# zarrs/zarrs

Hardware: AMD Instinct MI355X
Metric: decoded-array GiB/s, device-resident chunks, 1/2/4/8 MI355X; % HBM roofline (higher is better)
Workload: dtype f32; 1 GPU; C2: 4096 independent 64^3 f32 chunks per GPU, [transpose{order:[2,1,0]}, bytes{endian:big}], device-resident; chunks_per_gpu=4096, parallelism=chunk-partitioned x1

## Files before the change

include/zgpu.h:

```cpp
#ifndef ZGPU_H
#define ZGPU_H

#include <stdint.h>

#ifdef __cplusplus
extern "C" {
#endif

#define ZGPU_MAX_DIMS 8

enum {
  ZGPU_OK = 0,
  ZGPU_INVALID_CHECKSUM = 1,
  ZGPU_DECODED_SIZE_MISMATCH = 2,
  ZGPU_SHARD_INDEX_OOB = 3,
  ZGPU_CORRUPT_STREAM = 4,
  ZGPU_INVALID_BYTE_RANGE = 5,
  ZGPU_UNSUPPORTED = 6,
  ZGPU_CRC_INPUT_TOO_SHORT = 7,
  ZGPU_SHARD_TOO_SMALL = 8,
  ZGPU_SHUFFLE_LENGTH = 9,
  ZGPU_INVALID_ARGUMENT = 10,
  ZGPU_HIP_ERROR = 11,
  ZGPU_STORAGE_ERROR = 12,
// ... 46 lines not shown
  uint64_t shape[ZGPU_MAX_DIMS];
} zgpu_out_view;

#define ZGPU_COALESCE 0x20u

int zgpu_decode_into(zgpu_chain *chain, uint32_t ndim, const zgpu_chunk_desc *descs, uint64_t n,
                     const zgpu_out_view *view, uint32_t flags, int32_t *status, void *hip_stream);

typedef struct zgpu_result zgpu_result;
int zgpu_decode_pinned(zgpu_chain *chain, uint32_t ndim, const zgpu_chunk_desc *descs, uint64_t n,
                       const uint64_t *out_shape, uint32_t flags, int32_t *status, const void **data,
                       zgpu_result **result);
void zgpu_result_release(zgpu_result *result);

int zgpu_ctx_set_coalescing(zgpu_ctx *ctx, uint32_t window_us, uint32_t max_calls, uint64_t max_bytes);
int zgpu_ctx_coalescing_stats(const zgpu_ctx *ctx, uint64_t *batches, uint64_t *calls);

int zgpu_plan_create(zgpu_chain *chain, uint32_t ndim, const zgpu_chunk_desc *descs, uint64_t n,
                     const uint64_t *out_shape, uint32_t flags, zgpu_plan **out);
int zgpu_plan_execute(zgpu_plan *plan, void *out, int32_t *status, void *hip_stream);
int zgpu_plan_status(zgpu_plan *plan, int32_t *status, void *hip_stream);
void zgpu_plan_destroy(zgpu_plan *plan);
uint64_t zgpu_plan_algorithmic_bytes(const zgpu_plan *plan);

typedef struct zgpu_group zgpu_group;
int zgpu_group_create(zgpu_chain *const *chains, uint32_t ndim, uint32_t n_parts, const zgpu_chunk_desc *const *descs,
                      const uint64_t *n_descs, const uint64_t *const *out_shapes, uint32_t flags, zgpu_group **out);
int zgpu_group_execute(zgpu_group *group, void *const *outs, int32_t *status, void *hip_stream);
int zgpu_group_status(zgpu_group *group, int32_t *status, void *hip_stream);
uint32_t zgpu_group_layout(const zgpu_group *group, uint32_t *lane_of, uint32_t *part_of, uint32_t *lits_first,
                           uint32_t n);
uint64_t zgpu_group_algorithmic_bytes(const zgpu_group *group);
uint32_t zgpu_group_counters(const zgpu_group *group, uint64_t *out, uint32_t n);
void zgpu_group_destroy(zgpu_group *group);

#define ZGPU_CTR_ENC_BYTES 0
#define ZGPU_CTR_ZSTD_SERIAL 1
#define ZGPU_CTR_ZSTD_PARALLEL 2
#define ZGPU_CTR_BLOSC_RERUN 3
#define ZGPU_CTR_BLOSC_BLOCKS 4
#define ZGPU_CTR_ITEMS 5
#define ZGPU_CTR_ZSTD_LATENCY 6
#define ZGPU_N_COUNTERS 7
uint32_t zgpu_plan_counters(const zgpu_plan *plan, uint64_t *out, uint32_t n);
uint32_t zgpu_last_counters(uint64_t *out, uint32_t n);

// ... 82 lines not shown
```

zarrs_amd/_lib.py:

```python
from __future__ import annotations

import ctypes as C
import os

HERE = os.path.dirname(os.path.abspath(__file__))
LIB_PATH = os.environ.get("ZGPU_LIB") or os.path.join(HERE, "lib", "libzgpu.so")
MAX_DIMS = 8

STATUS_NAMES = [
    "OK", "INVALID_CHECKSUM", "DECODED_SIZE_MISMATCH", "SHARD_INDEX_OOB", "CORRUPT_STREAM",
    "INVALID_BYTE_RANGE", "UNSUPPORTED", "CRC_INPUT_TOO_SHORT", "SHARD_TOO_SMALL", "SHUFFLE_LENGTH",
    "INVALID_ARGUMENT", "HIP_ERROR", "STORAGE_ERROR",
]
OK, INVALID_CHECKSUM, DECODED_SIZE_MISMATCH, SHARD_INDEX_OOB, CORRUPT_STREAM, INVALID_BYTE_RANGE, \
    UNSUPPORTED, CRC_INPUT_TOO_SHORT, SHARD_TOO_SMALL, SHUFFLE_LENGTH, INVALID_ARGUMENT, HIP_ERROR, \
    STORAGE_ERROR = range(13)

ENC_DEVICE = 0x1
OUT_DEVICE = 0x2
ONE_STREAM = 0x10
ZSTD_LITS_FIRST = 0x40
NO_VALIDATE = 0x4
DIRECT_IO = 0x8
COALESCE = 0x20
WHOLE = (1 << 64) - 1

EXPORTS = [
    "zgpu_ctx_create", "zgpu_ctx_destroy", "zgpu_last_error", "zgpu_status_name", "zgpu_version",
    "zgpu_chain_create", "zgpu_chain_destroy", "zgpu_chain_element_size", "zgpu_decode_batch",
    "zgpu_plan_create", "zgpu_plan_execute", "zgpu_plan_status", "zgpu_plan_destroy", "zgpu_plan_algorithmic_bytes",
    "zgpu_retrieve_array_subset", "zgpu_decode_files", "zgpu_retrieve_array_subset_files",
    "zgpu_chain_encoded_size", "zgpu_encode_batch", "zgpu_plan_counters", "zgpu_last_counters",
    "zgpu_last_size_mismatch", "zgpu_cache_create", "zgpu_cache_destroy", "zgpu_cache_clear", "zgpu_cache_stats",
    "zgpu_cache_retrieve_array_subset", "zgpu_retrieve_array_subset_dlpack", "zgpu_chain_encoded_bound",
    "zgpu_encode_chunks", "zgpu_retrieve_array_subset_multi", "zgpu_decode_into", "zgpu_ctx_set_coalescing",
    "zgpu_ctx_coalescing_stats", "zgpu_ctx_refcount", "zgpu_decode_pinned", "zgpu_result_release",
    "zgpu_encode_pinned", "zgpu_ctx_release_cached", "zgpu_ctx_pool_stats",
    "zgpu_group_create", "zgpu_group_execute", "zgpu_group_status", "zgpu_group_layout",
    "zgpu_group_algorithmic_bytes", "zgpu_group_counters", "zgpu_group_destroy",
]
CTR_ENC_BYTES, CTR_ZSTD_SERIAL, CTR_ZSTD_PARALLEL, CTR_BLOSC_RERUN, CTR_BLOSC_BLOCKS, CTR_ITEMS, \
    CTR_ZSTD_LATENCY = range(7)
N_COUNTERS = 7


class ChunkDesc(C.Structure):
    _fields_ = [
        ("enc", C.c_void_p),
        ("enc_len", C.c_uint64),
        ("chunk_shape", C.c_uint64 * MAX_DIMS),
        ("sel_start", C.c_uint64 * MAX_DIMS),
        ("sel_shape", C.c_uint64 * MAX_DIMS),
        ("out_start", C.c_uint64 * MAX_DIMS),
    ]


class OutView(C.Structure):
    _fields_ = [
        ("base", C.c_void_p),
        ("array_shape", C.c_uint64 * MAX_DIMS),
        ("start", C.c_uint64 * MAX_DIMS),
        ("shape", C.c_uint64 * MAX_DIMS),
    ]
# ... 63 lines not shown
    L.zgpu_ctx_refcount.argtypes = [vp]
    L.zgpu_ctx_refcount.restype = C.c_int64
    L.zgpu_last_error.restype = C.c_char_p
    L.zgpu_last_error.argtypes = [vp]
    L.zgpu_status_name.restype = C.c_char_p
    L.zgpu_status_name.argtypes = [i32]
    L.zgpu_version.restype = C.c_char_p
    L.zgpu_chain_create.argtypes = [vp, C.c_char_p, C.c_char_p, vp, u32, i32, C.POINTER(vp)]
    L.zgpu_chain_destroy.argtypes = [vp]
    L.zgpu_chain_element_size.restype = u32
    L.zgpu_chain_element_size.argtypes = [vp]
    L.zgpu_decode_batch.argtypes = [vp, u32, C.POINTER(ChunkDesc), u64, vp, P64, u32,
                                    C.POINTER(C.c_int32), vp]
    L.zgpu_decode_into.argtypes = [vp, u32, C.POINTER(ChunkDesc), u64, C.POINTER(OutView), u32,
                                   C.POINTER(C.c_int32), vp]
    L.zgpu_ctx_set_coalescing.argtypes = [vp, u32, u32, u64]
    L.zgpu_ctx_coalescing_stats.argtypes = [vp, P64, P64]
    L.zgpu_plan_create.argtypes = [vp, u32, C.POINTER(ChunkDesc), u64, P64, u32, C.POINTER(vp)]
    L.zgpu_plan_execute.argtypes = [vp, vp, C.POINTER(C.c_int32), vp]
    L.zgpu_plan_status.argtypes = [vp, C.POINTER(C.c_int32), vp]
    L.zgpu_plan_destroy.argtypes = [vp]
    L.zgpu_plan_algorithmic_bytes.restype = u64
    L.zgpu_plan_algorithmic_bytes.argtypes = [vp]
    L.zgpu_group_create.argtypes = [C.POINTER(vp), u32, u32, C.POINTER(C.POINTER(ChunkDesc)), P64, C.POINTER(P64),
                                    u32, C.POINTER(vp)]
    L.zgpu_group_execute.argtypes = [vp, C.POINTER(vp), C.POINTER(C.c_int32), vp]
    L.zgpu_group_status.argtypes = [vp, C.POINTER(C.c_int32), vp]
    L.zgpu_group_layout.restype = u32
    L.zgpu_group_layout.argtypes = [vp, C.POINTER(u32), C.POINTER(u32), C.POINTER(u32), u32]
    L.zgpu_group_algorithmic_bytes.restype = u64
    L.zgpu_group_algorithmic_bytes.argtypes = [vp]
    L.zgpu_group_counters.restype = u32
    L.zgpu_group_counters.argtypes = [vp, P64, u32]
    L.zgpu_group_destroy.argtypes = [vp]
    L.zgpu_retrieve_array_subset.argtypes = [vp, u32, P64, P64, C.POINTER(vp), P64, P64, P64, vp,
                                             u32, vp]
    L.zgpu_decode_files.argtypes = [vp, u32, C.POINTER(ChunkDesc), C.POINTER(FileRange), u64, vp, P64,
                                    u32, C.POINTER(C.c_int32), vp]
    L.zgpu_retrieve_array_subset_files.argtypes = [vp, u32, P64, P64, C.POINTER(C.c_char_p), P64, P64,
                                                   vp, u32, vp]
    L.zgpu_chain_encoded_size.restype = C.c_int64
    L.zgpu_chain_encoded_size.argtypes = [vp, u32, P64]
    L.zgpu_encode_batch.argtypes = [vp, u32, P64, vp, P64, C.POINTER(EncodeDesc), u64, u32, vp]
    L.zgpu_chain_encoded_bound.restype = C.c_int64
    L.zgpu_chain_encoded_bound.argtypes = [vp, u32, P64]
    L.zgpu_encode_chunks.argtypes = [vp, u32, P64, vp, P64, C.POINTER(EncodeDesc), u64, u32, P64, vp]
# ... 45 lines not shown
```

zarrs_amd/csrc/kernels/dev.hpp:

```cpp
#pragma once
#include <hip/hip_runtime.h>

#include <cstdint>

namespace zgpu {

__device__ __forceinline__ uint32_t swap_word(uint32_t x, uint32_t comp) {
  if (comp == 4) return __builtin_bswap32(x);
  if (comp == 2) return ((x >> 8) & 0x00FF00FFu) | ((x << 8) & 0xFF00FF00u);
  return x;
}

__device__ __forceinline__ uint4 swap_vec(uint4 v, uint32_t comp) {
  if (comp == 8) return make_uint4(__builtin_bswap32(v.y), __builtin_bswap32(v.x),
                                   __builtin_bswap32(v.w), __builtin_bswap32(v.z));
  return make_uint4(swap_word(v.x, comp), swap_word(v.y, comp), swap_word(v.z, comp),
                    swap_word(v.w, comp));
}

typedef unsigned int zg_v4u __attribute__((ext_vector_type(4)));
__device__ __forceinline__ uint4 nt_load16(const void *p) {
  const zg_v4u x = __builtin_nontemporal_load((const zg_v4u *)p);
  return make_uint4(x.x, x.y, x.z, x.w);
}
__device__ __forceinline__ void nt_store16(void *p, uint4 v) {
  const zg_v4u x = {v.x, v.y, v.z, v.w};
  __builtin_nontemporal_store(x, (zg_v4u *)p);
}

}
```

zarrs_amd/csrc/kernels/launch.hpp:

```cpp
#pragma once
#include <hip/hip_runtime.h>

#include "../common.hpp"

#include <cstdlib>

namespace zgpu {

inline uint64_t max_grid_blocks(uint32_t threads) {
  uint64_t m = (0xFFFFFFFFull / threads) & ~(uint64_t)0xFFF;
  if (const char *e = std::getenv("ZGPU_MAX_GRID")) {
    const uint64_t v = std::strtoull(e, nullptr, 10);
    if (v && v < m) m = v;
  }
  return m;
}

inline uint32_t device_cu_count() {
  static uint32_t cache[64] = {0};
  int dev = 0;
  if (hipGetDevice(&dev) != hipSuccess || dev < 0 || dev >= 64) return 256;
  if (!cache[dev]) {
    int n = 0;
    if (hipDeviceGetAttribute(&n, hipDeviceAttributeMultiprocessorCount, dev) != hipSuccess || n <= 0) n = 256;
    cache[dev] = (uint32_t)n;
  }
  return cache[dev];
}

enum ScatterMode : uint32_t { SCATTER_ROWS = 0, SCATTER_TILED = 1, SCATTER_GENERIC = 2 };
constexpr __host__ __device__ int tiled_slabs(uint32_t es) { return es == 8 ? 2 : 4; }

hipError_t launch_scatter(const ZgItem *items, const uint64_t *geom, uint32_t *status, const ZgScatter &P,
                          uint8_t *out, uint32_t n_items, uint32_t mode, uint64_t units_per_item,
                          hipStream_t s, uint32_t *live_scratch = nullptr);
uint64_t scatter_units_per_item(uint32_t mode, const ZgScatter &P, const uint64_t *max_sel_shape);

struct ZgBoxCopy {
  uint32_t outer, pad0;
  uint64_t shape[ZG_MAXD], src_stride[ZG_MAXD], dst_stride[ZG_MAXD];
  uint64_t src_base, dst_base, run_bytes, n_runs;
};
hipError_t launch_box_copy(const uint8_t *src, uint8_t *dst, const ZgBoxCopy &P, hipStream_t s);

hipError_t launch_crc32c_strip(ZgItem *items, uint32_t *status, uint32_t n_items, int at_start, int verify,
                               hipStream_t s);

enum : uint32_t { CK_ADLER32 = 0, CK_FLETCHER32 = 1 };
uint64_t linsum_scratch_bytes(uint32_t n_items, uint64_t len_hint);
hipError_t launch_linsum_strip(uint32_t kind, ZgItem *items, uint32_t *status, uint32_t n_items, int at_start,
                               int verify, uint64_t len_hint, void *scratch, hipStream_t s);

struct ZgIndexSpec {
  uint64_t n_inner;
  uint64_t index_bytes;
  uint32_t at_start;
  uint32_t big_endian;
  uint32_t n_crc;
  uint32_t crc_at_start[4];
// ... 188 lines not shown
```

zarrs_amd/csrc/kernels/scatter.hip:

```cpp
#include <hip/hip_runtime.h>

#include <algorithm>

#include "../common.hpp"
#include "launch.hpp"
#include "dev.hpp"

namespace zgpu {

__device__ __forceinline__ uint4 load_elem(const uint8_t *p, uint32_t es, uint32_t comp, uint32_t swap) {
  uint8_t b[16];
  uintptr_t a = (uintptr_t)p;
  if (es == 4 && (a & 3) == 0) {
    uint32_t w = *(const uint32_t *)p;
    if (swap) w = swap_word(w, comp);
    return make_uint4(w, 0, 0, 0);
  }
  if (es == 2 && (a & 1) == 0) {
    uint32_t w = *(const uint16_t *)p;
    if (swap) w = ((w >> 8) | (w << 8)) & 0xFFFFu;
    return make_uint4(w, 0, 0, 0);
  }
  if (es == 8 && (a & 7) == 0) {
    uint2 w = *(const uint2 *)p;
// ... 241 lines not shown
  rows_unit(items, geom, status, P, out, (uint32_t)(bid / blocks_per_item), (uint32_t)(bid % blocks_per_item));
}

__global__ void k_live_items(const ZgItem *__restrict__ items, const uint32_t *__restrict__ status, uint32_t n,
                             uint32_t *__restrict__ list, uint32_t *__restrict__ count) {
  const uint32_t i = blockIdx.x * blockDim.x + threadIdx.x;
  if (i < n && !status[i] && !(items[i].flags & ZG_ITEM_DIRECT)) list[atomicAdd(count, 1u)] = i;
}

__global__ __launch_bounds__(SCATTER_THREADS) void k_scatter_rows_list(
    const ZgItem *__restrict__ items, const uint64_t *__restrict__ geom, uint32_t *__restrict__ status,
    ZgScatter P, uint8_t *__restrict__ out, uint32_t blocks_per_item, const uint32_t *__restrict__ list,
    const uint32_t *__restrict__ count) {
  const uint64_t total = (uint64_t)*count * blocks_per_item;
  for (uint64_t w = blockIdx.x; w < total; w += gridDim.x) {
    __syncthreads();
    rows_unit(items, geom, status, P, out, list[w / blocks_per_item], (uint32_t)(w % blocks_per_item));
  }
}

constexpr int TILE = 64;

template <int ES>
__global__ __launch_bounds__(SCATTER_THREADS) void k_scatter_tiled(
    const ZgItem *__restrict__ items, const uint64_t *__restrict__ geom, uint32_t *__restrict__ status,
    ZgScatter P, uint8_t *__restrict__ out, uint32_t tiles_per_item, uint64_t block_base) {
  using T = typename std::conditional<ES == 1, uint8_t, typename std::conditional<ES == 2, uint16_t,
            typename std::conditional<ES == 4, uint32_t, uint2>::type>::type>::type;
  constexpr int TJ = tiled_slabs(ES);
  constexpr int PITCH = TILE + (ES >= 4 ? 1 : 4 / ES);
  constexpr int SLAB = TILE * PITCH + (ES >= 4 ? 1 : 4 / ES);
  __shared__ T tile[TJ * SLAB];
  const uint64_t bid = block_base + blockIdx.x;
  const uint32_t item = (uint32_t)(bid / tiles_per_item);
  uint32_t t = (uint32_t)(bid % tiles_per_item);
  const ZgItem it = items[item];
  if (!item_live(it, status, item, P)) return;
  const uint32_t nd = P.nd, A = P.tile_a, Lx = nd - 1, B = P.tile_b;
  const uint64_t *g = geom + (uint64_t)item * 3 * nd;
  const uint64_t *ss = g, *sh = g + nd, *os = g + 2 * nd;
  const bool hasB = B < nd;
  const uint64_t bext = hasB ? sh[B] : 1;
  const uint32_t nta = (uint32_t)((sh[A] + TILE - 1) / TILE), ntl = (uint32_t)((sh[Lx] + TILE - 1) / TILE);
  const uint32_t nbg = (uint32_t)((bext + TJ - 1) / TJ);
  const uint32_t ta = t % nta; t /= nta;
  const uint32_t tl = t % ntl; t /= ntl;
  const uint32_t tb = t % nbg; t /= nbg;
  uint64_t so = 0, dof = 0, rem = t;
  for (int d = (int)nd - 1; d >= 0; d--) {
    if ((uint32_t)d == A || (uint32_t)d == Lx || (uint32_t)d == B) continue;
    const uint64_t c = rem % sh[d];
    rem /= sh[d];
    so += (ss[d] + c) * P.enc_stride[d];
    dof += (os[d] + c) * P.out_stride[d];
  }
  if (rem) return;
  const uint64_t a0 = (uint64_t)ta * TILE, l0 = (uint64_t)tl * TILE, b0 = (uint64_t)tb * TJ;
  const uint32_t na = (uint32_t)min<uint64_t>(TILE, sh[A] - a0), nl = (uint32_t)min<uint64_t>(TILE, sh[Lx] - l0);
  const uint32_t nb = (uint32_t)min<uint64_t>(TJ, bext - b0);
  const uint64_t sL = P.enc_stride[Lx], dA = P.out_stride[A];
  const uint64_t sB = hasB ? P.enc_stride[B] : 0, dB = hasB ? P.out_stride[B] : 0;
  so += (ss[A] + a0) * P.enc_stride[A] + (ss[Lx] + l0) * sL + (hasB ? (ss[B] + b0) * sB : 0);
  dof += (os[A] + a0) * dA + (os[Lx] + l0) + (hasB ? (os[B] + b0) * dB : 0);
  T *dst = (T *)(out) + dof;
  constexpr int VPR = TILE * ES / 16;
  constexpr int EPV = 16 / ES;
  constexpr int NV = TJ * TILE * VPR;
  const bool oaligned = (((uint64_t)dst & 15) == 0) && ((dA * ES) % 16 == 0) && ((dB * ES) % 16 == 0) &&
                        nl == TILE;
  if (it.flags & ZG_ITEM_FILL) {
    T fv;
    __builtin_memcpy(&fv, P.fill, ES);
    if (oaligned) {
      uint4 x;
      T *xe = (T *)&x;
#pragma unroll
      for (int k = 0; k < EPV; k++) xe[k] = fv;
      for (uint32_t e = threadIdx.x; e < (uint32_t)NV; e += SCATTER_THREADS) {
        const uint32_t a = e / (TJ * VPR), jj = (e / VPR) % TJ, v = e % VPR;
        if (a < na && jj < nb) nt_store16(dst + jj * dB + (uint64_t)a * dA + v * EPV, x);
      }
    } else {
      for (uint32_t e = threadIdx.x; e < (uint32_t)(TJ * TILE * TILE); e += SCATTER_THREADS) {
        const uint32_t a = e / (TJ * TILE), jj = (e / TILE) % TJ, l = e % TILE;
        if (a < na && jj < nb && l < nl) dst[jj * dB + (uint64_t)a * dA + l] = fv;
      }
    }
    return;
  }
  const T *src = (const T *)(it.src) + so;
  const uint32_t swap = P.swap && P.comp > 1;
  const bool aligned = (((uint64_t)src & 15) == 0) && ((sL * ES) % 16 == 0) && ((sB * ES) % 16 == 0) &&
                       na == TILE;
  if (aligned) {
    constexpr int PER = NV / SCATTER_THREADS;
    uint4 x[PER];
#pragma unroll
    for (int p = 0; p < PER; p++) {
      const uint32_t e = p * SCATTER_THREADS + threadIdx.x;
      const uint32_t l = e / (TJ * VPR), jj = (e / VPR) % TJ, v = e % VPR;
      if (l < nl && jj < nb) x[p] = nt_load16(src + jj * sB + (uint64_t)l * sL + v * EPV);
    }
#pragma unroll
    for (int p = 0; p < PER; p++) {
      const uint32_t e = p * SCATTER_THREADS + threadIdx.x;
      const uint32_t l = e / (TJ * VPR), jj = (e / VPR) % TJ, v = e % VPR;
      if (l < nl && jj < nb) {
        uint4 y = swap ? swap_vec(x[p], P.comp) : x[p];
        const T *ye = (const T *)&y;
#pragma unroll
        for (int k = 0; k < EPV; k++) tile[jj * SLAB + l * PITCH + v * EPV + k] = ye[k];
      }
    }
  } else {
    for (uint32_t e = threadIdx.x; e < (uint32_t)(TJ * TILE * TILE); e += SCATTER_THREADS) {
      const uint32_t l = e / (TJ * TILE), jj = (e / TILE) % TJ, a = e % TILE;
      if (l < nl && jj < nb && a < na) {
        uint4 y = load_elem((const uint8_t *)(src + jj * sB + (uint64_t)l * sL + a), ES, P.comp, swap);
        T v;
        __builtin_memcpy(&v, &y, ES);
        tile[jj * SLAB + l * PITCH + a] = v;
      }
    }
  }
  __syncthreads();
  if (oaligned) {
#pragma unroll
    for (int p = 0; p < NV / SCATTER_THREADS; p++) {
      const uint32_t e = p * SCATTER_THREADS + threadIdx.x;
      const uint32_t a = e / (TJ * VPR), jj = (e / VPR) % TJ, v = e % VPR;
      if (a < na && jj < nb) {
        uint4 y;
        T *ye = (T *)&y;
#pragma unroll
        for (int k = 0; k < EPV; k++) ye[k] = tile[jj * SLAB + (v * EPV + k) * PITCH + a];
        nt_store16(dst + jj * dB + (uint64_t)a * dA + v * EPV, y);
      }
    }
  } else {
    for (uint32_t e = threadIdx.x; e < (uint32_t)(TJ * TILE * TILE); e += SCATTER_THREADS) {
      const uint32_t a = e / (TJ * TILE), jj = (e / TILE) % TJ, l = e % TILE;
      if (a < na && jj < nb && l < nl) dst[jj * dB + (uint64_t)a * dA + l] = tile[jj * SLAB + l * PITCH + a];
    }
  }
}

__global__ __launch_bounds__(SCATTER_THREADS) void k_scatter_generic(
    const ZgItem *__restrict__ items, const uint64_t *__restrict__ geom, uint32_t *__restrict__ status,
    ZgScatter P, uint8_t *__restrict__ out, uint32_t blocks_per_item, uint64_t block_base) {
  const uint64_t bid = block_base + blockIdx.x;
  const uint32_t item = (uint32_t)(bid / blocks_per_item);
  const uint32_t blk = (uint32_t)(bid % blocks_per_item);
  const ZgItem it = items[item];
  if (!item_live(it, status, item, P)) return;
  const uint32_t nd = P.nd, es = P.es;
  const uint64_t *g = geom + (uint64_t)item * 3 * nd;
  uint64_t n = 1;
  for (uint32_t d = 0; d < nd; d++) n *= g[nd + d];
  const uint64_t e = (uint64_t)blk * SCATTER_THREADS + threadIdx.x;
  if (e >= n) return;
  uint64_t rem = e, so = 0, dof = 0;
  for (int d = (int)nd - 1; d >= 0; d--) {
    const uint64_t c = rem % g[nd + d];
    rem /= g[nd + d];
    so += (g[d] + c) * P.enc_stride[d];
// ... 69 lines not shown

uint64_t scatter_units_per_item(uint32_t mode, const ZgScatter &P, const uint64_t *max_sel_shape) {
  const uint32_t nd = P.nd;
  if (mode == SCATTER_ROWS) {
    uint64_t rows = 1;
    for (uint32_t d = 0; d + 1 < nd; d++) rows *= max_sel_shape[d];
    return (rows + ROWS_PER_BLOCK - 1) / ROWS_PER_BLOCK;
  }
  if (mode == SCATTER_TILED) {
    const uint64_t tj = tiled_slabs(P.es);
    uint64_t t = 1;
    for (uint32_t d = 0; d < nd; d++) {
      if (d == P.tile_a || d == nd - 1) t *= (max_sel_shape[d] + TILE - 1) / TILE;
      else if (d == P.tile_b) t *= (max_sel_shape[d] + tj - 1) / tj;
      else t *= max_sel_shape[d];
    }
    return t;
  }
  uint64_t n = 1;
  for (uint32_t d = 0; d < nd; d++) n *= max_sel_shape[d];
  return (n + SCATTER_THREADS - 1) / SCATTER_THREADS;
}

}

namespace zgpu {

__global__ __launch_bounds__(64) void k_box_copy(const uint8_t *__restrict__ src, uint8_t *__restrict__ dst,
                                                   ZgBoxCopy P) {
  const uint32_t lane = threadIdx.x & 63;
  const uint64_t waves = (uint64_t)gridDim.x * (blockDim.x >> 6);
  for (uint64_t r = (uint64_t)blockIdx.x * (blockDim.x >> 6) + (threadIdx.x >> 6); r < P.n_runs; r += waves) {
    uint64_t k = r, so = 0, dof = 0;
    for (int d = (int)P.outer - 1; d >= 0; d--) {
      const uint64_t c = k % P.shape[d];
      k /= P.shape[d];
      so += c * P.src_stride[d];
      dof += c * P.dst_stride[d];
    }
    const uint8_t *s = src + P.src_base + so;
    uint8_t *t = dst + P.dst_base + dof;
    const uint64_t n = P.run_bytes;
    if ((((uintptr_t)s | (uintptr_t)t | n) & 15) == 0) {
      for (uint64_t i = (uint64_t)lane * 16; i < n; i += 64 * 16)
        *(uint4 *)(t + i) = *(const uint4 *)(s + i);
    } else if ((((uintptr_t)s | (uintptr_t)t | n) & 3) == 0) {
// ... 17 lines not shown
```

zarrs_amd/csrc/zgpu.cpp:

```cpp
#include <hip/hip_runtime.h>

#include <algorithm>
#include <atomic>
#include <chrono>
#include <cstdio>
#include <cstdlib>
#include <cstring>
#include <condition_variable>
#include <map>
#include <memory>
#include <mutex>
#include <string>
#include <vector>

#include "../../include/zgpu.h"
#include "chain.hpp"
#include "common.hpp"
#include "kernels/launch.hpp"
#include "fsstore.hpp"
#include "internal.hpp"
#include "xfer.hpp"

using namespace zgpu;

// ... 307 lines not shown
    Z.ev_done = zev2[1];
  }
  struct Grow {
    void *p = nullptr;
    size_t n = 0;
  };
  Grow bl_info, bl_bases, bl_subs, bl_sub_status, bl_sub_kind, bl_blocks, bl_tmp, bl_zblks, bl_znblk, bl_zmode,
      bl_zlit, bl_zseq, bl_zaux, bl_zser, bl_lzl, bl_zseg, bl_zrec, bl_zalias, bl_znorm, gz_crc, live_list,
      ck_parts;
  uint64_t in_len_hint = 0;
  uint8_t *bl_h = nullptr;
  size_t bl_h_n = 0;
  void *grow(Grow &g, size_t bytes) {
    if (g.n < bytes) {
      ctx->dev_free(g.p);
      g.p = ctx->dev_alloc(bytes);
      g.n = bytes;
    }
    return g.p;
  }
  unsigned long long *d_counter = nullptr;
  uint8_t *d_ctl = nullptr, *h_ctl = nullptr;
  size_t ctl_bytes = 0;
  uint8_t *d_enc_stage = nullptr;
  uint64_t last_enc_bytes = 0;
  uint64_t last_counters[CTR_N] = {};
  uint8_t *last_out = nullptr;
  BlCaps bl_caps{};
  bool bl_caps_valid = false, bl_caps_seen = false;
  bool bl_direct = false;
  bool gz_direct = false;
  GzDirect gz{};
  std::vector<uint64_t> bl_need;
  uint64_t *d_bl_need = nullptr;
  bool zstd_serial_off = false, zstd_serial_skipped = false;
  uint32_t *d_zser = nullptr;
  uint32_t *d_order = nullptr;
  uint32_t *d_gz_seg = nullptr;
  bool no_scatter = false;

  ~zgpu_plan() {
    if (!ctx) return;
    struct Unref {
      zgpu_ctx *c;
      ~Unref() { ctx_unref(c); }
    } unref{ctx};
    if (own.stream) {
      (void)hipStreamSynchronize(own.stream);
      (void)hipStreamDestroy(own.stream);
    }
    if (own.order_ev) (void)hipEventDestroy(own.order_ev);
    void *bufs[] = {d_items, d_items_init, d_geom, d_shards, d_index, d_shard_status, d_mids, d_mids_init,
                    d_mid_status, d_shard_status2, d_mid_shards, d_index2, d_bl_need,
                    d_pool[0], d_pool[1], zs.blks, zs.nblk, zs.mode, zs.lit, zs.seq, d_ctl,
                    d_enc_stage, d_zser, d_order, d_gz_seg, zs.lit_rec, zs.ext, zs.ext_cnt, zs.norm};
    for (void *b : bufs) ctx->dev_free(b);
    if (zside) {
      (void)hipStreamSynchronize(zside);
      (void)hipStreamDestroy(zside);
    }
    if (zs2) {
      (void)hipStreamSynchronize(zs2);
      (void)hipStreamDestroy(zs2);
    }
    for (hipEvent_t e : zev2)
      if (e) (void)hipEventDestroy(e);
    for (hipEvent_t e : zev)
      if (e) (void)hipEventDestroy(e);
    for (Grow *g : {&bl_info, &bl_bases, &bl_subs, &bl_sub_status, &bl_sub_kind, &bl_blocks, &bl_tmp, &bl_zblks,
                    &bl_znblk, &bl_zmode, &bl_zlit, &bl_zseq, &bl_zaux, &bl_zser, &bl_lzl, &bl_zseg, &bl_zrec, &bl_zalias,
                    &bl_znorm, &gz_crc, &live_list, &ck_parts})
      ctx->dev_free(g->p);
    ctx->host_free(bl_h);
    ctx->host_free(h_ctl);
  }
};

static void reset_call_state() {
// ... 335 lines not shown
    s *= eshape[a];
  }
  for (uint32_t a = 0; a < nd; a++) S.enc_stride[m[a]] = est[a];
  for (uint32_t d = 0; d < nd; d++) {
    S.chunk_shape[d] = leaf_shape[d];
    S.out_stride[d] = out_strides[mo[d]];
  }
  S.tile_a = m[nd - 1];
  S.tile_b = ZG_MAXD;
  for (uint32_t d = 0; d + 1 < nd; d++) {
    if (d == S.tile_a) continue;
    if (S.tile_b == ZG_MAXD || S.enc_stride[d] <= S.enc_stride[S.tile_b]) S.tile_b = d;
  }
  if (outer_perm && S.out_stride[nd - 1] != 1) {
    P.scatter_mode = SCATTER_GENERIC;
  } else if (S.tile_a == nd - 1) {
    P.scatter_mode = SCATTER_ROWS;
  } else if (!S.shuffle && (S.es == 1 || S.es == 2 || S.es == 4 || S.es == 8)) {
    P.scatter_mode = SCATTER_TILED;
  } else {
    P.scatter_mode = SCATTER_GENERIC;
  }
  P.scatter_units = P.items.empty() ? 0 : scatter_units_per_item(P.scatter_mode, S, max_sel);

  if (!P.stages.empty() && P.stages.back().kind == ST_BLOSC && P.scatter_mode == SCATTER_ROWS && !S.swap &&
      !S.shuffle && S.nelem > 0 && S.out_stride[nd - 1] == 1 && (S.chunk_shape[nd - 1] * S.es) % 16 == 0) {
    bool ok = true;
    uint64_t st = 1;
    for (int a = (int)nd - 1; a >= 0 && ok; a--) {
      ok = S.enc_stride[a] == st && (a == (int)nd - 1 || (S.out_stride[a] * S.es) % 16 == 0);
      st *= S.chunk_shape[a];
    }
    for (size_t i = 0; i < P.items.size() && ok; i++) {
      if (P.items[i].flags & ZG_ITEM_FILL) continue;
      const uint64_t *g = P.geom.data() + i * 3 * nd;
      for (uint32_t d = 0; d < nd && ok; d++) ok = g[d] == 0 && g[nd + d] == S.chunk_shape[d];
      ok = ok && (g[2 * nd + nd - 1] * S.es) % 16 == 0;
    }
    P.bl_direct = ok && !std::getenv("ZGPU_BLOSC_NO_DIRECT");
  }
  {
    const char *gz_env = std::getenv("ZGPU_GZIP_DIRECT");
    const bool gz_on = !gz_env || std::atoi(gz_env) != 0;
    const uint64_t Lb = S.chunk_shape[nd - 1] * S.es;
    bool ok = gz_on && !P.stages.empty() && P.stages.back().kind == ST_GZIP && P.scatter_mode == SCATTER_ROWS &&
              !S.swap && !S.shuffle && S.nelem > 0 && nd >= 1 && nd <= 3 && S.out_stride[nd - 1] == 1 && Lb >= 16 &&
// ... 77 lines not shown
        if (ni * P.slot_bytes <= par_max) {
          P.zs.ext = (uint32_t *)C.dev_alloc(2 * ni * P.slot_bytes * 4);
          P.zs.ext_cnt = (unsigned long long *)C.dev_alloc(ZEXT_ROUNDS * 8);
          P.zs.ext_items = ni;
        }
      }
    }
  }
  P.in_len_hint = 0;
  if (P.sharded) {
    uint64_t shard_max = 0;
    for (const ZgShard &sh : P.shards) shard_max = std::max(shard_max, sh.len);
    const int64_t b = P.leaf ? chain_encoded_bound(*P.leaf, P.scatter.nelem) : -1;
    P.in_len_hint = b >= 0 ? std::min<uint64_t>((uint64_t)b, shard_max) : shard_max;
  } else {
    for (const ZgItem &it : P.items) P.in_len_hint = std::max(P.in_len_hint, it.len);
  }
  for (const Stage &s : P.stages)
    if (ni && (s.kind == ST_ADLER32 || s.kind == ST_FLETCHER32))
      P.grow(P.ck_parts, linsum_scratch_bytes((uint32_t)ni, std::max(P.in_len_hint, P.slot_bytes)));
  P.ctl_bytes = 256 + ni * 4;
  P.d_ctl = (uint8_t *)C.dev_alloc(P.ctl_bytes);
  P.h_ctl = (uint8_t *)C.host_alloc(P.ctl_bytes);
  P.d_counter = (unsigned long long *)P.d_ctl;
  P.d_status = (uint32_t *)(P.d_ctl + 256);
  P.zs.counters = P.d_counter + CTR_ZSTD_SERIAL;
  P.zs.lat_count = P.d_counter + CTR_ZSTD_LATENCY;
  P.zs.ser_count = P.d_counter + CTR_ZSTD_NSER;
  P.zs.max_nblk = P.d_counter + CTR_ZSTD_MAXBLK;
  if (const char *e = std::getenv("ZGPU_ZSTD_FORCE_SERIAL")) P.zs.force_serial = std::atoi(e) != 0;
  if (!P.shards.empty()) {
    P.d_shards = (ZgShard *)C.dev_alloc(P.shards.size() * sizeof(ZgShard));
    P.d_index = (uint64_t *)C.dev_alloc(P.shards.size() * P.ispec.n_inner * 16);
    P.d_shard_status = (uint32_t *)C.dev_alloc(P.shards.size() * 4);
    HIPCHK(hipMemcpyAsync(P.d_shards, P.shards.data(), P.shards.size() * sizeof(ZgShard), hipMemcpyHostToDevice,
                          us));
  }
  if (!P.mids.empty()) {
    const size_t nm = P.mids.size();
    P.d_mids = (ZgItem *)C.dev_alloc(nm * sizeof(ZgItem));
    P.d_mids_init = (ZgItem *)C.dev_alloc(nm * sizeof(ZgItem));
    P.d_mid_status = (uint32_t *)C.dev_alloc(nm * 4);
    P.d_shard_status2 = (uint32_t *)C.dev_alloc(nm * 4);
    P.d_mid_shards = (ZgShard *)C.dev_alloc(nm * sizeof(ZgShard));
    P.d_index2 = (uint64_t *)C.dev_alloc(nm * P.ispec2.n_inner * 16);
    HIPCHK(hipMemcpyAsync(P.d_mids_init, P.mids.data(), nm * sizeof(ZgItem), hipMemcpyHostToDevice, us));
// ... 176 lines not shown
        wrote_direct = wrote_direct || direct;
      }
        crc_tail = 0;
        break;
      case ST_ZSTD:
        P.zstd_fork(P.zs, s);
        P.zs.lits_first = (P.flags & ZGPU_ZSTD_LITS_FIRST) && !P.zs.side ? 1u : 0u;
        HIPCHK(launch_zstd(P.d_items, P.d_status, ni, P.d_pool[st.pool], P.slot_bytes, P.zs, s));
        break;
      case ST_BLOSC:
        blosc_stage(P, st, out, s);
        break;
      case ST_UNSHUFFLE:
        HIPCHK(launch_unshuffle(P.d_items, P.d_status, ni, P.d_pool[st.pool], P.slot_bytes, st.elementsize, s));
        break;
    }
    if (!strips_only(st.kind)) len_hint = P.slot_bytes;
  }
  if (!P.no_scatter) {
    const char *le = std::getenv("ZGPU_SCATTER_LIST");
    uint32_t *live = nullptr;
    if (wrote_direct && le && std::atoi(le) != 0)
      live = (uint32_t *)P.grow(P.live_list, ((size_t)ni + 1) * 4);
    HIPCHK(launch_scatter(items, P.d_geom, P.d_status, P.scatter, out, ni, P.scatter_mode, P.scatter_units, s, live));
  }
}

static void size_detail(zgpu_plan &P, uint64_t d, const uint32_t *st, hipStream_t s) {
  const size_t ni = P.items.size();
  for (size_t i = 0; i < ni; i++) {
    if (P.items[i].desc != d || st[i] != ZGPU_DECODED_SIZE_MISMATCH) continue;
    const bool mutates = P.sharded || !P.stages.empty();
    ZgItem it{};
    HIPCHK(hipMemcpyAsync(&it, (mutates ? P.d_items : P.d_items_init) + i, sizeof(ZgItem), hipMemcpyDeviceToHost, s));
    HIPCHK(hipStreamSynchronize(s));
    bool materialised = false, exact = true;
    for (const Stage &stg : P.stages)
      if (!strips_only(stg.kind)) materialised = true;
    if (materialised) {
      exact = false;
      for (int k = 0; k < P.n_pools; k++) {
        const uint64_t lo = (uint64_t)P.d_pool[k], hi = lo + ni * P.slot_bytes;
        if (it.src >= lo && it.src < hi) exact = true;
      }
    }
    g_size_detail.valid = 1;
    g_size_detail.desc = d;
// ... 719 lines not shown
  reset_call_state();
  plan_enqueue(*P, (uint8_t *)out, s);
  if (!status) return ZGPU_OK;
  return plan_statuses(*P, status, s);
  ABI_GUARD_END
}

int zgpu_plan_status(zgpu_plan *P, int32_t *status, void *stream) {
  ABI_GUARD_BEGIN
  if (!P) return set_err(ZGPU_INVALID_ARGUMENT, "NULL argument");
  std::lock_guard<std::mutex> lk(P->mu);
  HIPCHK(hipSetDevice(P->ctx->device));
  const int rc = plan_statuses(*P, status, stream ? (hipStream_t)stream : plan_lane(*P)->stream);
  if (rc) set_err(rc, zgpu_status_name(rc));
  return rc;
  ABI_GUARD_END
}

void zgpu_plan_destroy(zgpu_plan *P) {
  if (!P) return;
  { std::lock_guard<std::mutex> lk(P->mu); }
  delete P;
}

uint64_t zgpu_plan_algorithmic_bytes(const zgpu_plan *P) { return P ? P->alg_bytes_static + P->last_enc_bytes : 0; }

uint32_t zgpu_plan_counters(const zgpu_plan *P, uint64_t *out, uint32_t n) {
  if (!P || !out) return 0;
  const uint32_t k = std::min<uint32_t>(n, CTR_N);
  std::memcpy(out, P->last_counters, k * sizeof(uint64_t));
  return k;
}

int zgpu_last_size_mismatch(uint64_t *desc, uint64_t *len, uint64_t *expected_len) {
  if (!g_size_detail.valid) return 0;
  if (desc) *desc = g_size_detail.desc;
  if (len) *len = g_size_detail.len;
  if (expected_len) *expected_len = g_size_detail.expected;
  return 1;
}

uint32_t zgpu_last_counters(uint64_t *out, uint32_t n) {
  if (!out) return 0;
  const uint32_t k = std::min<uint32_t>(n, CTR_N);
  std::memcpy(out, g_last_counters, k * sizeof(uint64_t));
  return k;
// ... 1535 lines not shown
```

Measured before the change: 2668 GiB/s.

## Add persistent software-pipelined tiled transpose scatter kernel for full-chunk selections

Adds a persistent grid-stride variant of the tiled transpose scatter, used when every chunk is fully selected and the strides are aligned. It precomputes per-item output origins on the host, prefetches item metadata, and overlaps the global loads for the next tile with the LDS stores of the current one. Unaligned, fill and mismatched items fall back to the old per-tile routine. This aims to cut per-block launch and index overhead and to hide memory latency, at the cost of more code paths, higher register use and an extra device buffer.

After: 2770 GiB/s (median of 6 runs). 1.04x the previous value.

```diff
diff --git a/include/zgpu.h b/include/zgpu.h
--- a/include/zgpu.h
+++ b/include/zgpu.h
@@ -92,6 +92,11 @@
 int zgpu_plan_status(zgpu_plan *plan, int32_t *status, void *hip_stream);
 void zgpu_plan_destroy(zgpu_plan *plan);
 uint64_t zgpu_plan_algorithmic_bytes(const zgpu_plan *plan);
+#define ZGPU_SCATTER_ROWS 0u
+#define ZGPU_SCATTER_TILED 1u
+#define ZGPU_SCATTER_GENERIC 2u
+#define ZGPU_SCATTER_TILED_PERSISTENT 3u
+uint32_t zgpu_plan_scatter_path(const zgpu_plan *plan);
 
 typedef struct zgpu_group zgpu_group;
 int zgpu_group_create(zgpu_chain *const *chains, uint32_t ndim, uint32_t n_parts, const zgpu_chunk_desc *const *descs,
diff --git a/zarrs_amd/_lib.py b/zarrs_amd/_lib.py
--- a/zarrs_amd/_lib.py
+++ b/zarrs_amd/_lib.py
@@ -37,8 +37,9 @@
     "zgpu_ctx_coalescing_stats", "zgpu_ctx_refcount", "zgpu_decode_pinned", "zgpu_result_release",
     "zgpu_encode_pinned", "zgpu_ctx_release_cached", "zgpu_ctx_pool_stats",
     "zgpu_group_create", "zgpu_group_execute", "zgpu_group_status", "zgpu_group_layout",
-    "zgpu_group_algorithmic_bytes", "zgpu_group_counters", "zgpu_group_destroy",
+    "zgpu_group_algorithmic_bytes", "zgpu_group_counters", "zgpu_group_destroy", "zgpu_plan_scatter_path",
 ]
+SCATTER_ROWS, SCATTER_TILED, SCATTER_GENERIC, SCATTER_TILED_PERSISTENT = range(4)
 CTR_ENC_BYTES, CTR_ZSTD_SERIAL, CTR_ZSTD_PARALLEL, CTR_BLOSC_RERUN, CTR_BLOSC_BLOCKS, CTR_ITEMS, \
     CTR_ZSTD_LATENCY = range(7)
 N_COUNTERS = 7
@@ -148,6 +149,8 @@
     L.zgpu_plan_destroy.argtypes = [vp]
     L.zgpu_plan_algorithmic_bytes.restype = u64
     L.zgpu_plan_algorithmic_bytes.argtypes = [vp]
+    L.zgpu_plan_scatter_path.restype = u32
+    L.zgpu_plan_scatter_path.argtypes = [vp]
     L.zgpu_group_create.argtypes = [C.POINTER(vp), u32, u32, C.POINTER(C.POINTER(ChunkDesc)), P64, C.POINTER(P64),
                                     u32, C.POINTER(vp)]
     L.zgpu_group_execute.argtypes = [vp, C.POINTER(vp), C.POINTER(C.c_int32), vp]
diff --git a/zarrs_amd/csrc/kernels/dev.hpp b/zarrs_amd/csrc/kernels/dev.hpp
--- a/zarrs_amd/csrc/kernels/dev.hpp
+++ b/zarrs_amd/csrc/kernels/dev.hpp
@@ -23,6 +23,11 @@
   const zg_v4u x = __builtin_nontemporal_load((const zg_v4u *)p);
   return make_uint4(x.x, x.y, x.z, x.w);
 }
+__device__ __forceinline__ uint4 nt_load16_g(const void *p) {
+  typedef const zg_v4u __attribute__((address_space(1))) *gptr;
+  const zg_v4u x = __builtin_nontemporal_load((gptr)(uintptr_t)p);
+  return make_uint4(x.x, x.y, x.z, x.w);
+}
 __device__ __forceinline__ void nt_store16(void *p, uint4 v) {
   const zg_v4u x = {v.x, v.y, v.z, v.w};
   __builtin_nontemporal_store(x, (zg_v4u *)p);
diff --git a/zarrs_amd/csrc/kernels/launch.hpp b/zarrs_amd/csrc/kernels/launch.hpp
--- a/zarrs_amd/csrc/kernels/launch.hpp
+++ b/zarrs_amd/csrc/kernels/launch.hpp
@@ -35,6 +35,21 @@
                           uint8_t *out, uint32_t n_items, uint32_t mode, uint64_t units_per_item,
                           hipStream_t s, uint32_t *live_scratch = nullptr);
 uint64_t scatter_units_per_item(uint32_t mode, const ZgScatter &P, const uint64_t *max_sel_shape);
+
+struct ZgTiledP {
+  uint32_t upi;
+  uint32_t nta, ntl, nbg;
+  uint32_t bext;
+  uint32_t sL, sB, dA, dB;
+  uint32_t nrest;
+  uint32_t rext[ZG_MAXD], rs[ZG_MAXD], rd[ZG_MAXD];
+};
+bool tiled_persistent_params(const ZgScatter &P, const uint64_t *geom, size_t n_items, ZgTiledP &Q,
+                             uint64_t *origin);
+hipError_t launch_scatter_tiled_p(const ZgItem *items, const uint64_t *geom, uint32_t *status, const uint64_t *origin,
+                                  const ZgScatter &P, const ZgTiledP &Q, uint8_t *out, uint32_t n_items,
+                                  uint32_t grid_cap, hipStream_t s);
+bool tiled_persistent_fits(uint64_t n_items, uint64_t upi);
 
 struct ZgBoxCopy {
   uint32_t outer, pad0;
diff --git a/zarrs_amd/csrc/kernels/scatter.hip b/zarrs_amd/csrc/kernels/scatter.hip
--- a/zarrs_amd/csrc/kernels/scatter.hip
+++ b/zarrs_amd/csrc/kernels/scatter.hip
@@ -287,18 +287,25 @@
 constexpr int TILE = 64;
 
 template <int ES>
-__global__ __launch_bounds__(SCATTER_THREADS) void k_scatter_tiled(
-    const ZgItem *__restrict__ items, const uint64_t *__restrict__ geom, uint32_t *__restrict__ status,
-    ZgScatter P, uint8_t *__restrict__ out, uint32_t tiles_per_item, uint64_t block_base) {
+struct Tiled {
   using T = typename std::conditional<ES == 1, uint8_t, typename std::conditional<ES == 2, uint16_t,
             typename std::conditional<ES == 4, uint32_t, uint2>::type>::type>::type;
-  constexpr int TJ = tiled_slabs(ES);
-  constexpr int PITCH = TILE + (ES >= 4 ? 1 : 4 / ES);
-  constexpr int SLAB = TILE * PITCH + (ES >= 4 ? 1 : 4 / ES);
-  __shared__ T tile[TJ * SLAB];
-  const uint64_t bid = block_base + blockIdx.x;
-  const uint32_t item = (uint32_t)(bid / tiles_per_item);
-  uint32_t t = (uint32_t)(bid % tiles_per_item);
+  static constexpr int TJ = tiled_slabs(ES);
+  static constexpr int PITCH = TILE + (ES >= 4 ? 1 : 4 / ES);
+  static constexpr int SLAB = TILE * PITCH + (ES >= 4 ? 1 : 4 / ES);
+  static constexpr int VPR = TILE * ES / 16;
+  static constexpr int EPV = 16 / ES;
+  static constexpr int NV = TJ * TILE * VPR;
+  static constexpr int PER = NV / SCATTER_THREADS;
+};
+
+template <int ES>
+__device__ __forceinline__ void tiled_unit(const ZgItem *__restrict__ items, const uint64_t *__restrict__ geom,
+                                           uint32_t *__restrict__ status, const ZgScatter &P,
+                                           uint8_t *__restrict__ out, typename Tiled<ES>::T *tile, uint32_t item,
+                                           uint32_t t) {
+  using T = typename Tiled<ES>::T;
+  constexpr int TJ = Tiled<ES>::TJ, PITCH = Tiled<ES>::PITCH, SLAB = Tiled<ES>::SLAB;
   const ZgItem it = items[item];
   if (!item_live(it, status, item, P)) return;
   const uint32_t nd = P.nd, A = P.tile_a, Lx = nd - 1, B = P.tile_b;
@@ -328,9 +335,7 @@
   so += (ss[A] + a0) * P.enc_stride[A] + (ss[Lx] + l0) * sL + (hasB ? (ss[B] + b0) * sB : 0);
   dof += (os[A] + a0) * dA + (os[Lx] + l0) + (hasB ? (os[B] + b0) * dB : 0);
   T *dst = (T *)(out) + dof;
-  constexpr int VPR = TILE * ES / 16;
-  constexpr int EPV = 16 / ES;
-  constexpr int NV = TJ * TILE * VPR;
+  constexpr int VPR = Tiled<ES>::VPR, EPV = Tiled<ES>::EPV, NV = Tiled<ES>::NV;
   const bool oaligned = (((uint64_t)dst & 15) == 0) && ((dA * ES) % 16 == 0) && ((dB * ES) % 16 == 0) &&
                         nl == TILE;
   if (it.flags & ZG_ITEM_FILL) {
@@ -364,7 +369,7 @@
     for (int p = 0; p < PER; p++) {
       const uint32_t e = p * SCATTER_THREADS + threadIdx.x;
       const uint32_t l = e / (TJ * VPR), jj = (e / VPR) % TJ, v = e % VPR;
-      if (l < nl && jj < nb) x[p] = nt_load16(src + jj * sB + (uint64_t)l * sL + v * EPV);
+      if (l < nl && jj < nb) x[p] = nt_load16_g(src + jj * sB + (uint64_t)l * sL + v * EPV);
     }
 #pragma unroll
     for (int p = 0; p < PER; p++) {
@@ -406,6 +411,182 @@
     for (uint32_t e = threadIdx.x; e < (uint32_t)(TJ * TILE * TILE); e += SCATTER_THREADS) {
       const uint32_t a = e / (TJ * TILE), jj = (e / TILE) % TJ, l = e % TILE;
       if (a < na && jj < nb && l < nl) dst[jj * dB + (uint64_t)a * dA + l] = tile[jj * SLAB + l * PITCH + a];
+    }
+  }
+}
+
+template <int ES>
+__global__ __launch_bounds__(SCATTER_THREADS) void k_scatter_tiled(
+    const ZgItem *__restrict__ items, const uint64_t *__restrict__ geom, uint32_t *__restrict__ status,
+    ZgScatter P, uint8_t *__restrict__ out, uint32_t tiles_per_item, uint64_t block_base) {
+  __shared__ typename Tiled<ES>::T tile[Tiled<ES>::TJ * Tiled<ES>::SLAB];
+  const uint64_t bid = block_base + blockIdx.x;
+  tiled_unit<ES>(items, geom, status, P, out, tile, (uint32_t)(bid / tiles_per_item),
+                 (uint32_t)(bid % tiles_per_item));
+}
+
+template <int ES>
+__global__ __launch_bounds__(SCATTER_THREADS, 2) void k_scatter_tiled_p(
+    const ZgItem *__restrict__ items, const uint64_t *__restrict__ geom, uint32_t *__restrict__ status,
+    const uint64_t *__restrict__ origin, ZgScatter P, ZgTiledP Q, uint8_t *__restrict__ out, uint32_t n_units) {
+  using T = typename Tiled<ES>::T;
+  constexpr int TJ = Tiled<ES>::TJ, PITCH = Tiled<ES>::PITCH, SLAB = Tiled<ES>::SLAB;
+  constexpr int VPR = Tiled<ES>::VPR, EPV = Tiled<ES>::EPV, PER = Tiled<ES>::PER;
+  __shared__ T tile[TJ * SLAB];
+  enum : uint32_t { SKIP = 0, FAST = 1, SLOW = 2, MISMATCH = 3 };
+  struct Raw {
+    uint64_t src, len, org;
+    uint32_t flags, st;
+  };
+  struct Unit {
+    const T *src;
+    T *dst;
+    uint32_t nb, kind, item, t;
+  };
+  const uint64_t want = P.nelem * ES;
+  auto fetch = [&](uint32_t u) {
+    const uint32_t item = u / Q.upi;
+    Raw r;
+    r.src = items[item].src;
+    r.len = items[item].len;
+    r.flags = items[item].flags;
+    r.st = status[item];
+    r.org = origin[item];
+    return r;
+  };
+  auto resolve = [&](const Raw &r, uint32_t u) {
+    Unit U;
+    U.item = u / Q.upi;
+    uint32_t t = u - U.item * Q.upi;
+    U.t = t;
+    U.src = nullptr;
+    U.dst = nullptr;
+    U.nb = 0;
+    if (r.st || (r.flags & ZG_ITEM_DIRECT)) {
+      U.kind = SKIP;
+      return U;
+    }
+    if (!(r.flags & ZG_ITEM_FILL) && r.len != want) {
+      U.kind = MISMATCH;
+      return U;
+    }
+    if ((r.flags & ZG_ITEM_FILL) || (r.src & 15)) {
+      U.kind = SLOW;
+      return U;
+    }
+    const uint32_t ta = t % Q.nta; t /= Q.nta;
+    const uint32_t tl = t % Q.ntl; t /= Q.ntl;
+    const uint32_t tb = t % Q.nbg; t /= Q.nbg;
+    uint32_t so = ta * TILE + tl * TILE * Q.sL + tb * TJ * Q.sB;
+    uint32_t dof = ta * TILE * Q.dA + tl * TILE + tb * TJ * Q.dB;
+    for (uint32_t k = 0; k < Q.nrest; k++) {
+      const uint32_t c = t % Q.rext[k];
+      t /= Q.rext[k];
+      so += c * Q.rs[k];
+      dof += c * Q.rd[k];
+    }
+    U.kind = FAST;
+    U.nb = min((uint32_t)TJ, Q.bext - tb * TJ);
+    U.src = (const T *)r.src + so;
+    U.dst = (T *)out + r.org + dof;
+    return U;
+  };
+  uint4 x[PER];
+  constexpr uint32_t RSTEP = SCATTER_THREADS / (TJ * VPR);
+  const uint32_t r0 = threadIdx.x / (TJ * VPR), jj = (threadIdx.x / VPR) % TJ, v = threadIdx.x % VPR;
+  auto load = [&](const Unit &U) {
+    const T *q = U.src + min(jj, U.nb - 1) * Q.sB + r0 * Q.sL + v * EPV;
+#pragma unroll
+    for (int p = 0; p < PER; p++, q += RSTEP * Q.sL) x[p] = nt_load16_g(q);
+  };
+  auto to_lds = [&](auto cc) {
+    constexpr uint32_t COMP = decltype(cc)::value;
+#pragma unroll
+    for (int p = 0; p < PER; p++) {
+      const uint32_t l = p * RSTEP + r0;
+      const uint4 y = COMP > 1 ? swap_vec(x[p], COMP) : x[p];
+      const T *ye = (const T *)&y;
+#pragma unroll
+      for (int k = 0; k < EPV; k++) tile[jj * SLAB + l * PITCH + v * EPV + k] = ye[k];
+    }
+  };
+  auto store = [&](const Unit &U) {
+    T *q = U.dst + min(jj, U.nb - 1) * Q.dB + r0 * Q.dA + v * EPV;
+#pragma unroll
+    for (int p = 0; p < PER; p++, q += RSTEP * Q.dA) {
+      const uint32_t a = p * RSTEP + r0;
+      uint4 y;
+      T *ye = (T *)&y;
+#pragma unroll
+      for (int k = 0; k < EPV; k++) ye[k] = tile[jj * SLAB + (v * EPV + k) * PITCH + a];
+      nt_store16(q, y);
+    }
+  };
+  const uint32_t first = blockIdx.x, step = gridDim.x, end = n_units;
+  uint32_t any_slow = 0;
+  auto aside = [&](const Unit &U) {
+    if (U.kind == SLOW) any_slow = 1;
+    if (U.kind == MISMATCH && threadIdx.x == 0) status[U.item] = ZG_DECODED_SIZE_MISMATCH;
+  };
+  auto run = [&](auto cc) {
+    uint32_t un = first;
+    Raw ahead = fetch(min(un, end - 1));
+    while (un < end) {
+      Unit cur = resolve(ahead, un);
+      un += step;
+      ahead = fetch(min(un, end - 1));
+      if (cur.kind != FAST) {
+        aside(cur);
+        continue;
+      }
+      load(cur);
+      Unit nxt{};
+      bool more = un < end;
+      if (more) {
+        nxt = resolve(ahead, un);
+        un += step;
+        ahead = fetch(min(un, end - 1));
+      }
+      to_lds(cc);
+      __syncthreads();
+      for (;;) {
+        if (nxt.kind != FAST) {
+          store(cur);
+          __syncthreads();
+          if (more) aside(nxt);
+          break;
+        }
+        load(nxt);
+        store(cur);
+        Unit nn{};
+        const bool more2 = un < end;
+        if (more2) {
+          nn = resolve(ahead, un);
+          un += step;
+          ahead = fetch(min(un, end - 1));
+        }
+        __syncthreads();
+        to_lds(cc);
+        __syncthreads();
+        cur = nxt;
+        nxt = nn;
+        more = more2;
+      }
+    }
+  };
+  switch (P.swap ? P.comp : 1u) {
+    case 2: run(std::integral_constant<uint32_t, 2>{}); break;
+    case 4: run(std::integral_constant<uint32_t, 4>{}); break;
+    case 8: run(std::integral_constant<uint32_t, 8>{}); break;
+    default: run(std::integral_constant<uint32_t, 1>{});
+  }
+  if (any_slow) {
+    for (uint32_t u = first; u < end; u += step) {
+      const uint32_t item = u / Q.upi;
+      if ((items[item].flags & ZG_ITEM_FILL) || (items[item].src & 15)) {
+        tiled_unit<ES>(items, geom, status, P, out, tile, item, u - item * Q.upi);
+        __syncthreads();
+      }
     }
   }
 }
@@ -521,6 +702,83 @@
   return (n + SCATTER_THREADS - 1) / SCATTER_THREADS;
 }
 
+bool tiled_persistent_params(const ZgScatter &P, const uint64_t *geom, size_t n_items, ZgTiledP &Q,
+                             uint64_t *origin) {
+  const uint32_t nd = P.nd, A = P.tile_a, Lx = nd - 1, B = P.tile_b, es = P.es;
+  if (!n_items || A >= nd || A == Lx || P.shuffle || !P.nelem || P.nelem >= (1ull << 32)) return false;
+  if (es != 1 && es != 2 && es != 4 && es != 8) return false;
+  if (P.enc_stride[A] != 1 || P.out_stride[Lx] != 1) return false;
+  if (P.chunk_shape[A] % TILE || P.chunk_shape[Lx] % TILE) return false;
+  uint64_t span = 0;
+  for (uint32_t d = 0; d < nd; d++) {
+    const uint64_t ext = P.chunk_shape[d];
+    span += (ext - 1) * P.out_stride[d];
+    if (ext > 1 && d != A && (P.enc_stride[d] * es) % 16) return false;
+    if (ext > 1 && d != Lx && (P.out_stride[d] * es) % 16) return false;
+  }
+  if (span >= (1ull << 32)) return false;
+  for (size_t i = 0; i < n_items; i++) {
+    const uint64_t *g = geom + i * 3 * nd;
+    uint64_t o = 0;
+    for (uint32_t d = 0; d < nd; d++) {
+      if (g[d] != 0 || g[nd + d] != P.chunk_shape[d]) return false;
+      o += g[2 * nd + d] * P.out_stride[d];
+    }
+    if ((o * es) % 16) return false;
+    origin[i] = o;
+  }
+  const bool hasB = B < nd;
+  const uint32_t tj = (uint32_t)tiled_slabs(es);
+  Q = ZgTiledP{};
+  Q.nta = (uint32_t)(P.chunk_shape[A] / TILE);
+  Q.ntl = (uint32_t)(P.chunk_shape[Lx] / TILE);
+  Q.bext = hasB ? (uint32_t)P.chunk_shape[B] : 1;
+  Q.nbg = (Q.bext + tj - 1) / tj;
+  Q.sL = (uint32_t)P.enc_stride[Lx];
+  Q.dA = (uint32_t)P.out_stride[A];
+  Q.sB = Q.bext > 1 ? (uint32_t)P.enc_stride[B] : 0;
+  Q.dB = Q.bext > 1 ? (uint32_t)P.out_stride[B] : 0;
+  uint64_t upi = (uint64_t)Q.nta * Q.ntl * Q.nbg;
+  for (int d = (int)nd - 1; d >= 0; d--) {
+    if ((uint32_t)d == A || (uint32_t)d == Lx || (uint32_t)d == B) continue;
+    const uint32_t k = Q.nrest++;
+    Q.rext[k] = (uint32_t)P.chunk_shape[d];
+    Q.rs[k] = Q.rext[k] > 1 ? (uint32_t)P.enc_stride[d] : 0;
+    Q.rd[k] = Q.rext[k] > 1 ? (uint32_t)P.out_stride[d] : 0;
+    upi *= Q.rext[k];
+  }
+  if (upi >= (1ull << 32)) return false;
+  Q.upi = (uint32_t)upi;
+  return true;
+}
+
+bool tiled_persistent_fits(uint64_t n_items, uint64_t upi) { return n_items * upi < 0xFFFFFFFFull - (1u << 24); }
+
+template <int ES>
+static void launch_tiled_p(const ZgItem *items, const uint64_t *geom, uint32_t *status, const uint64_t *origin,
+                           const ZgScatter &P, const ZgTiledP &Q, uint8_t *out, uint32_t n_units, uint32_t grid_cap,
+                           hipStream_t s) {
+  uint64_t g = std::min<uint64_t>(n_units, max_grid_blocks(SCATTER_THREADS));
+  if (grid_cap) g = std::min<uint64_t>(g, grid_cap);
+  hipLaunchKernelGGL(k_scatter_tiled_p<ES>, dim3((uint32_t)g), dim3(SCATTER_THREADS), 0, s, items, geom, status, origin,
+                     P, Q, out, n_units);
+}
+
+hipError_t launch_scatter_tiled_p(const ZgItem *items, const uint64_t *geom, uint32_t *status, const uint64_t *origin,
+                                  const ZgScatter &P, const ZgTiledP &Q, uint8_t *out, uint32_t n_items,
+                                  uint32_t grid_cap, hipStream_t s) {
+  if (!n_items || !Q.upi || !tiled_persistent_fits(n_items, Q.upi)) return hipErrorInvalidConfiguration;
+  const uint32_t n_units = n_items * Q.upi;
+  switch (P.es) {
+    case 1: launch_tiled_p<1>(items, geom, status, origin, P, Q, out, n_units, grid_cap, s); break;
+    case 2: launch_tiled_p<2>(items, geom, status, origin, P, Q, out, n_units, grid_cap, s); break;
+    case 4: launch_tiled_p<4>(items, geom, status, origin, P, Q, out, n_units, grid_cap, s); break;
+    case 8: launch_tiled_p<8>(items, geom, status, origin, P, Q, out, n_units, grid_cap, s); break;
+    default: return hipErrorInvalidValue;
+  }
+  return hipGetLastError();
+}
+
 }
 
 namespace zgpu {
diff --git a/zarrs_amd/csrc/zgpu.cpp b/zarrs_amd/csrc/zgpu.cpp
--- a/zarrs_amd/csrc/zgpu.cpp
+++ b/zarrs_amd/csrc/zgpu.cpp
@@ -353,6 +353,11 @@
   unsigned long long *d_counter = nullptr;
   uint8_t *d_ctl = nullptr, *h_ctl = nullptr;
   size_t ctl_bytes = 0;
+  bool tiled_p = false;
+  ZgTiledP tiled_q{};
+  std::vector<uint64_t> origin;
+  uint64_t *d_origin = nullptr;
+  uint32_t last_path = SCATTER_GENERIC;
   uint8_t *d_enc_stage = nullptr;
   uint64_t last_enc_bytes = 0;
   uint64_t last_counters[CTR_N] = {};
@@ -384,7 +389,7 @@
     void *bufs[] = {d_items, d_items_init, d_geom, d_shards, d_index, d_shard_status, d_mids, d_mids_init,
                     d_mid_status, d_shard_status2, d_mid_shards, d_index2, d_bl_need,
                     d_pool[0], d_pool[1], zs.blks, zs.nblk, zs.mode, zs.lit, zs.seq, d_ctl,
-                    d_enc_stage, d_zser, d_order, d_gz_seg, zs.lit_rec, zs.ext, zs.ext_cnt, zs.norm};
+                    d_enc_stage, d_zser, d_order, d_gz_seg, zs.lit_rec, zs.ext, zs.ext_cnt, zs.norm, d_origin};
     for (void *b : bufs) ctx->dev_free(b);
     if (zside) {
       (void)hipStreamSynchronize(zside);
@@ -766,6 +771,13 @@
     P.scatter_mode = SCATTER_GENERIC;
   }
   P.scatter_units = P.items.empty() ? 0 : scatter_units_per_item(P.scatter_mode, S, max_sel);
+  if (P.scatter_mode == SCATTER_TILED && !P.items.empty()) {
+    P.origin.resize(P.items.size());
+    P.tiled_p = tiled_persistent_params(S, P.geom.data(), P.items.size(), P.tiled_q, P.origin.data()) &&
+                P.tiled_q.upi == P.scatter_units && tiled_persistent_fits(P.items.size(), P.tiled_q.upi);
+    if (!P.tiled_p) P.origin.clear();
+  }
+  P.last_path = P.tiled_p ? ZGPU_SCATTER_TILED_PERSISTENT : P.scatter_mode;
 
   if (!P.stages.empty() && P.stages.back().kind == ST_BLOSC && P.scatter_mode == SCATTER_ROWS && !S.swap &&
       !S.shuffle && S.nelem > 0 && S.out_stride[nd - 1] == 1 && (S.chunk_shape[nd - 1] * S.es) % 16 == 0) {
@@ -889,6 +901,10 @@
   P.ctl_bytes = 256 + ni * 4;
   P.d_ctl = (uint8_t *)C.dev_alloc(P.ctl_bytes);
   P.h_ctl = (uint8_t *)C.host_alloc(P.ctl_bytes);
+  if (P.tiled_p) {
+    P.d_origin = (uint64_t *)C.dev_alloc(ni * 8);
+    HIPCHK(hipMemcpyAsync(P.d_origin, P.origin.data(), ni * 8, hipMemcpyHostToDevice, us));
+  }
   P.d_counter = (unsigned long long *)P.d_ctl;
   P.d_status = (uint32_t *)(P.d_ctl + 256);
   P.zs.counters = P.d_counter + CTR_ZSTD_SERIAL;
@@ -1111,7 +1127,17 @@
     uint32_t *live = nullptr;
     if (wrote_direct && le && std::atoi(le) != 0)
       live = (uint32_t *)P.grow(P.live_list, ((size_t)ni + 1) * 4);
-    HIPCHK(launch_scatter(items, P.d_geom, P.d_status, P.scatter, out, ni, P.scatter_mode, P.scatter_units, s, live));
+    const char *pe = std::getenv("ZGPU_TILED_PERSIST");
+    const bool persist = P.tiled_p && (!pe || std::atoi(pe) != 0) && ((uintptr_t)out & 15) == 0;
+    if (persist) {
+      const char *ge = std::getenv("ZGPU_TILED_GRID");
+      const uint32_t cap = ge ? (uint32_t)std::strtoul(ge, nullptr, 10) : 0;
+      HIPCHK(launch_scatter_tiled_p(items, P.d_geom, P.d_status, P.d_origin, P.scatter, P.tiled_q, out, ni, cap, s));
+      P.last_path = ZGPU_SCATTER_TILED_PERSISTENT;
+    } else {
+      HIPCHK(launch_scatter(items, P.d_geom, P.d_status, P.scatter, out, ni, P.scatter_mode, P.scatter_units, s, live));
+      P.last_path = P.scatter_mode;
+    }
   }
 }
 
@@ -1877,6 +1903,8 @@
   { std::lock_guard<std::mutex> lk(P->mu); }
   delete P;
 }
+
+uint32_t zgpu_plan_scatter_path(const zgpu_plan *P) { return P ? P->last_path : ZGPU_SCATTER_GENERIC; }
 
 uint64_t zgpu_plan_algorithmic_bytes(const zgpu_plan *P) { return P ? P->alg_bytes_static + P->last_enc_bytes : 0; }
 
```
